# ntampellini/FIRECODE

Hardware: AMD Instinct MI355X
Metric: conformer-pair RMSD alignments/s (higher is better)
Workload: dtype f64

## Files before the change

### firecode_amd/_lib.py

```python

from __future__ import annotations

import ctypes as C
import os

import numpy as np

_HERE = os.path.dirname(os.path.abspath(__file__))
LIB_PATH = os.environ.get("FC_LIB_PATH") or os.path.join(_HERE, "libfc_hip.so")

FC_OK = 0
FC_E_INVALID, FC_E_NODEVICE, FC_E_HIP, FC_E_NOMEM, FC_E_LIMIT, FC_E_INTERNAL = -1, -2, -3, -4, -5, -6


class FirecodeHipError(RuntimeError):

    def __init__(self, code, message):
        super().__init__(f"libfc_hip error {code}: {message}")
        self.code = code


class FirecodeHipInputError(FirecodeHipError, ValueError):
    """FC_E_INVALID / FC_E_LIMIT: the arguments were rejected before any launch."""

# ... 76 lines not shown
    "fc_prune_export_pairs_dev": [_ens, C.c_void_p, _i64],
    "fc_prune_from_gathered_dev": [_ens, C.c_void_p, _i64, _i64, _i64, _p_u8, _p_i64],
    "fc_prune_from_gathered_dev_enqueue": [_ens, C.c_void_p, _i64, _i64, _i64, _i64, _i64],
    "fc_prune_collect": [_ens, _i64, _i64, _p_u8, _p_i64],
    "fc_stream_set": [C.c_void_p],
    "fc_memory_trim": [],
    "fc_host_alloc_pinned": [C.c_int64, C.POINTER(C.c_void_p)],
    "fc_host_free_pinned": [C.c_void_p],
    "fc_inertia_moments": [_p_f64, _i64, _i64, _p_f64, _p_f64],
    "fc_prune_rmsd_rot_corr": [_p_f64, _i64, _i64, _p_u8, _p_i64, _i64, _p_u8, _p_f64, C.POINTER(C.c_int32), _i64,
                               _f64, _f64, _p_f64, _f64, _i64, _p_u8, _p_u64],
    "fc_align_by_moi": [_p_f64, _i64, _i64, _p_f64, _p_f64],
    "fc_prune_moi": [_p_f64, _i64, _i64, _p_f64, _f64, _p_f64, _f64, _i64, _p_u8],
    "fc_moi_simbits": [_p_f64, _i64, _i64, _p_f64, _f64, _p_f64, _f64, _p_u64],
    "fc_align_to_first": [_p_f64, _i64, _i64, _p_i64, _i64, _p_f64],
    "fc_rototranslate": [_p_f64, _i64, _i64, _p_f64, _p_f64, _p_f64],
    "fc_clash_self": [_p_f64, _i64, _i64, _f64, _f64, _p_i64],
    "fc_clash_fragments": [_p_f64, _i64, _i64, _p_i64, _i64, _f64, _i64, _p_i64, _p_u8],
    "fc_clash_graph": [_p_f64, _i64, _i64, _p_u8, _f64, _p_i64],
    "fc_fitness_check": [_p_f64, _i64, _i64, _p_i64, _p_f64, _i64, _f64, _p_f64, _p_u8],
    "fc_bond_changes": [_p_f64, _i64, _i64, C.POINTER(C.c_int32), _i64, _p_f64, _p_f64, _i64, _p_u64, _p_i64, _p_i64,
                        _i64, _i64, _p_i64, _p_u8],
    "fc_bond_changes_list": [_p_f64, _i64, _i64, C.POINTER(C.c_int32), _i64, _p_f64, _p_f64, _i64, _p_u64, _p_i64,
                             _p_i64, _i64, _p_i64, _p_i64],
    "fc_embed_poses_clash": [_p_f64, _i64, _i64, _p_f64, _i64, _i64, _p_i64, _p_i64, _p_f64, _p_f64,
                             _p_f64, _p_f64, _i64, _f64, _i64, _p_i64, _p_u8, _p_f64],
    "fc_embed_mol_transforms": [_p_f64, _i64, _i64, _p_i64, _i64, _p_f64, _p_f64, _i64, _p_f64, _i64, _p_f64, _p_f64],
    "fc_embed_trimolecular": [C.POINTER(_p_f64), _p_i64, _p_i64, C.POINTER(_p_i64), _p_i64, _i64, _p_i64, _p_f64,
                              _p_f64, _p_f64, _p_f64, _p_u8, _p_i64, _p_f64, _p_f64, _i64, C.POINTER(C.c_int32),
                              _i64, _f64, _i64, _f64, _p_f64, _p_f64, _p_u8, _p_u8],
    "fc_embed_grid_clash": [_p_f64, _i64, _i64, _p_i64, _i64, _p_f64, _p_f64, _p_f64, _i64, _i64, _p_i64, _i64,
                            _p_f64, _p_f64, _p_f64, _i64, _p_f64, _i64, _f64, _i64, _p_u8,
                            C.POINTER(C.c_int32), _p_f64],
    "fc_embed_grid_dedupe": [_p_f64, _i64, _i64, _p_i64, _i64, _p_f64, _p_f64, _p_f64, _i64, _i64, _p_i64, _i64,
                             _p_f64, _p_f64, _p_f64, _i64, _p_f64, _i64, _f64, _i64, _f64, _p_u8, _p_u8],
    "fc_string_embed": [_p_f64, _i64, _i64, _p_f64, _p_f64, _i64, _p_f64, _i64, _i64, _p_f64, _p_f64, _i64, _p_f64, _i64,
                        _p_i64, _i64, _f64, _i64, _f64, _p_u8, _p_u8, _p_f64, _p_f64],
    "fc_torsion_scan": [_p_f64, _i64, _p_i64, _i64, _p_u8, _p_i64, _i64, _f64, _i64, _p_f64, _p_i64],
    "fc_torsion_scan_fingerprints": [_p_f64, _i64, _p_i64, _i64, _p_u8, _p_i64, _i64, _f64, _i64, _p_i64, _i64,
                                     _p_f64, _p_i64, _p_f64],
    "fc_torsion_scan_tfd": [_p_f64, _i64, _p_i64, _i64, _p_u8, _p_i64, _i64, _f64, _i64, _p_i64, _i64, _f64, _p_i64, _p_u8],
    "fc_torsion_scan_tfd_grid": [_p_f64, _i64, _p_i64, _i64, _p_u8, _p_i64, _p_i64, _f64, _i64, _p_i64, _i64, _f64, _p_i64, _p_u8],
    "fc_torsion_fingerprint": [_p_f64, _i64, _i64, _p_i64, _i64, _p_f64],
    "fc_tfd_simbits": [_p_f64, _i64, _i64, _f64, _i64, _i64, _p_u64],
    "fc_tfd_first_match": [_p_f64, _i64, _i64, _f64, _p_i64],
    "fc_tfd_last_form": [_p_i64],
    "fc_tfd_ladder_from_first_match": [_p_i64, _i64, _p_u8],
    "fc_tfd_prune": [_p_f64, _i64, _i64, _f64, _p_u8],
    "fc_debug_pyset_order_ints": [_p_i64, _i64, _p_i64, _p_i64],
    "fc_debug_pyset_order_pairs": [_p_i64, _i64, _p_i64, _p_i64],
    "fc_debug_pyset_order_pairs_device": [_p_i64, _i64, _p_i64],
    "fc_debug_tfd_ladder_emulate": [_p_i64, _i64, _p_u8],
    "fc_debug_ladder_from_pairs": [_p_u64, _i64, _i64, _i64, C.c_int, _i64, _p_u8, _p_i64],
    "fc_xyz_write": [C.c_char_p, C.POINTER(C.c_char_p), _i64, _p_f64, _i64, C.c_char_p, C.c_int],
    "fc_xyz_scan": [C.c_char_p, _p_i64, _p_i64],
    "fc_cartesian_product_i64": [_p_i64, _p_i64, _i64, _p_i64],
    "fc_cartesian_product_f64": [_p_f64, _p_i64, _i64, _p_f64],
    "fc_xyz_read": [C.c_char_p, _i64, _i64, C.c_char_p, _p_f64],
    "fc_bench_prune_rmsd": [_ens, _f64, _f64, _i64, _p_f64, _p_f64, _p_u8, _p_i64],
    "fc_stream_use": [C.c_void_p],
    "fc_ensemble_twin": [_ens, C.POINTER(_ens)],
    "fc_prune_rmsd_begin_split_async": [_ens, _f64, _f64, _i64, _i64, _i64, C.c_void_p, C.c_int],
    "fc_screen_last_kind": [],
    "fc_debug_screen_plan": [_i64, _i64, _i64, _i64, _f64, _f64, _i64, _p_i64],
    "fc_debug_mfma_f16_model": [_i64, _p_i64, _p_f64],
    "fc_debug_h2_covariance": [_ens, _i64, _i64, C.POINTER(C.c_float), _p_f64, _p_f64],
# ... 725 lines not shown
```

### firecode_amd/csrc/fc_api_geom.cpp

```cpp
#include "fc_internal.h"

using namespace fc;

extern "C" {

int fc_alignment_matrices(const double *p, const double *q, int64_t n_pairs, int64_t A,
                          double *M_out) {
  FC_API_LOCK;
  FC_REQUIRE(n_pairs >= 0 && A >= 1, "bad shape");
  if (n_pairs == 0) return FC_OK;
  FC_REQUIRE(p && q && M_out, "NULL pointer argument");
  FC_TRY(ensure_init());
  DevBuf dp, dq, dM;
  FC_TRY(upload(dp, p, (size_t)n_pairs * A * 3));
  FC_TRY(upload(dq, q, (size_t)n_pairs * A * 3));
  FC_TRY(dM.reserve((size_t)n_pairs * 9 * sizeof(double)));
  FC_TRY(launch_alignment_matrices(dp.as<double>(), dq.as<double>(), n_pairs, A, dM.as<double>()));
  FC_TRY(d2h(M_out, dM.p, (size_t)n_pairs * 9 * sizeof(double)));
  return sync();
}

int fc_align_by_moi(const double *coords, int64_t N, int64_t A, const double *masses, double *out) {
  FC_API_LOCK;
  FC_REQUIRE(N >= 0 && A >= 1, "bad shape");
// ... 362 lines not shown
    if (na1 * na2 * 4 * (int64_t)sizeof(int) > 64 * 1024)
      return set_error(FC_E_LIMIT, "na1*na2=%lld angle pairs per group exceed the 4096 of the LDS list",
                       (long long)(na1 * na2));
    FC_TRY(X2a.reserve(G2 * A2 * 3 * sizeof(double)));
    FC_TRY(dacc.reserve((size_t)P));
    FC_TRY(launch_embed_pretransform(d2.as<double>(), n2, A2, na2, R2.as<double>(), t2.as<double>(), 1, 0,
                                     X2a.as<double>()));
    FC_TRY(launch_embed_group_dedupe(X1.as<double>(), n1, A1, na1, X2a.as<double>(), n2, A2, na2, rmsd_thr,
                                     dpass.as<uint8_t>(), dacc.as<uint8_t>()));
    FC_TRY(d2h(accept_out, dacc.p, (size_t)P));
  }
  FC_TRY(d2h(pass_out, dpass.p, (size_t)P));
  if (counts_out) FC_TRY(d2h(counts_out, dcnt.p, (size_t)P * sizeof(int32_t)));
  FC_TRY(sync());
  if (ms_kernel) {
    float ms = 0.f;
    FC_HIP_TRY(hipEventElapsedTime(&ms, c.ev0, c.ev1));
    *ms_kernel = ms;
  }
  return FC_OK;
}

int fc_embed_grid_clash(const double *m1, int64_t n1, int64_t A1, const int64_t *reactive1,
                        int64_t nr1, const double *ps1, const double *pe1, const double *m2,
                        int64_t n2, int64_t A2, const int64_t *reactive2, int64_t nr2,
                        const double *ps2, const double *pe2, const double *angles1, int64_t na1,
                        const double *angles2, int64_t na2, double thresh, int64_t max_clashes,
                        uint8_t *pass_out, int32_t *counts_out, double *ms_kernel) {
  FC_API_LOCK;
  return embed_grid(m1, n1, A1, reactive1, nr1, ps1, pe1, m2, n2, A2, reactive2, nr2, ps2, pe2, angles1,
                    na1, angles2, na2, thresh, max_clashes, pass_out, counts_out, ms_kernel, 0.0, nullptr);
}

int fc_embed_grid_dedupe(const double *m1, int64_t n1, int64_t A1, const int64_t *reactive1,
                         int64_t nr1, const double *ps1, const double *pe1, const double *m2,
                         int64_t n2, int64_t A2, const int64_t *reactive2, int64_t nr2,
                         const double *ps2, const double *pe2, const double *angles1, int64_t na1,
                         const double *angles2, int64_t na2, double thresh, int64_t max_clashes,
                         double rmsd_thr, uint8_t *pass_out, uint8_t *accept_out) {
  FC_API_LOCK;
  FC_REQUIRE(accept_out != nullptr, "accept_out is NULL");
  return embed_grid(m1, n1, A1, reactive1, nr1, ps1, pe1, m2, n2, A2, reactive2, nr2, ps2, pe2, angles1,
                    na1, angles2, na2, thresh, max_clashes, pass_out, nullptr, nullptr, rmsd_thr, accept_out);
}

int fc_embed_trimolecular(const double *const coords[3], const int64_t n_conf[3], const int64_t n_atoms[3],
                          const int64_t *const reactive[3], const int64_t n_reactive[3], int64_t J,
                          const int64_t *conf, const double *piv_start, const double *piv_end,
                          const double *vecs, const double *dirs0, const uint8_t *run, const int64_t *rtab,
                          const double *norms, const double *ua, int64_t U, const int32_t *aidx, int64_t S,
                          double thresh, int64_t max_clashes, double rmsd_thr, double *dirs_out,
                          double *Rt_out, uint8_t *pass_out, uint8_t *accept_out) {
  FC_API_LOCK;
  FC_REQUIRE(coords && n_conf && n_atoms && reactive && n_reactive, "NULL pointer argument");
  FC_REQUIRE(J >= 0 && U >= 1 && S >= 1, "bad shape");
  if (J == 0) return FC_OK;
  FC_REQUIRE(conf && piv_start && piv_end && vecs && dirs0 && run && rtab && norms && ua && aidx && dirs_out &&
                 Rt_out && pass_out && accept_out,
             "NULL pointer argument");
  FC_REQUIRE(thresh > 0.0 && rmsd_thr > 0.0 && max_clashes >= 0, "thresholds must be positive");
  int64_t Atot = 0;
  for (int i = 0; i < 3; ++i) {
    FC_REQUIRE(coords[i] && reactive[i] && n_conf[i] >= 1 && n_atoms[i] >= 1, "bad molecule %d", i);
    FC_REQUIRE(n_reactive[i] >= 1 && n_reactive[i] <= 2, "molecule %d: 1 or 2 reactive atoms expected", i);
    for (int64_t r = 0; r < n_reactive[i]; ++r)
      FC_REQUIRE(reactive[i][r] >= 0 && reactive[i][r] < n_atoms[i], "reactive index out of range");
// ... 115 lines not shown
```

### firecode_amd/csrc/fc_embed.hip

```cpp
#include "fc_internal.h"
#include "fc_kabsch_math.h"

#include <algorithm>

namespace fc {

__device__ __forceinline__ void rot_axis_angle(double ax, double ay, double az, double angle_deg,
                                               double (&M)[9]) {
  double a2 = angle_deg / 2.0;
  a2 *= 3.141592653589793 / 180.0;
  double sn, cs;
  sincos(a2, &sn, &cs);
  const double nrm = sqrt((ax * ax + ay * ay) + az * az);
  const double q1 = sn * (ax / nrm), q2 = sn * (ay / nrm), q3 = sn * (az / nrm), q0 = cs;
  M[0] = 2.0 * (q0 * q0 + q1 * q1) - 1.0;
  M[1] = 2.0 * (q1 * q2 - q0 * q3);
  M[2] = 2.0 * (q1 * q3 + q0 * q2);
  M[3] = 2.0 * (q1 * q2 + q0 * q3);
  M[4] = 2.0 * (q0 * q0 + q2 * q2) - 1.0;
  M[5] = 2.0 * (q2 * q3 - q0 * q1);
  M[6] = 2.0 * (q1 * q3 - q0 * q2);
  M[7] = 2.0 * (q2 * q3 + q0 * q1);
  M[8] = 2.0 * (q0 * q0 + q3 * q3) - 1.0;
}
// ... 234 lines not shown
          const fc_f2 X = SX[ap], Y = SY[ap], Z = SZ[ap], Nn = SN[ap];
#pragma unroll
          for (int q = 0; q < NB; ++q) {
            fc_f2 v = __builtin_elementwise_fma(bz[q], Z, Nn);
            v = __builtin_elementwise_fma(by[q], Y, v);
            v = __builtin_elementwise_fma(bx[q], X, v);
            m[q] = fminf(fminf(m[q], v.x), v.y);
          }
        }
        if (scanning) {
#pragma unroll
          for (int q = NB - 1; q >= 0; --q)
            if (b0 + q < A2 && b0 + q >= resume && !(m[q] >= tb[q])) pending = b0 + q;
          if (pending < 0) resume = max(resume, min(b0 + NB, A2));
        }
      }
      if (pending >= 0) {
        const double ex = base2[(int64_t)(pending * 3 + 0) * S2 + s2];
        const double ey = base2[(int64_t)(pending * 3 + 1) * S2 + s2];
        const double ez = base2[(int64_t)(pending * 3 + 2) * S2 + s2];
        for (int a = 0; a < A1; ++a) {
          const double dx = ex - s[a * 3], dy = ey - s[a * 3 + 1], dz = ez - s[a * 3 + 2];
          const double d2 = ((dx * dx) + dy * dy) + dz * dz;
          cnt += (d2 < thr2) ? 1 : 0;
        }
        resume = (cnt > max_clashes) ? A2 : pending + 1;
      }
    }
    if (on) {
      const int64_t c2 = s2 / na2, a2 = s2 % na2;
      const int64_t p = ((c2 * n1 + c1) * 2 + o) * (na1 * na2) + (a2 * na1 + a1);
      pass[p] = (cnt <= max_clashes) ? 1 : 0;
      if (counts) counts[p] = cnt;
    }
  }
}

__global__ void __launch_bounds__(256)
k_string_transforms(const double *__restrict__ cen1, const double *__restrict__ vec1, int64_t n1,
                    int64_t K1, const double *__restrict__ cen2, const double *__restrict__ vec2,
                    int64_t n2, int64_t K2, const double *__restrict__ angles, int64_t nA,
                    double *__restrict__ R_out, double *__restrict__ t_out, int64_t *__restrict__ c1_out,
                    int64_t *__restrict__ c2_out) {
  const int64_t p = (int64_t)blockIdx.x * blockDim.x + threadIdx.x;
  const int64_t P = n1 * n2 * K1 * K2 * nA;
  if (p >= P) return;
  const int64_t ia = p % nA;
  const int64_t ki = (p / nA) % (K1 * K2);
  const int64_t ci = p / (nA * K1 * K2);
  const int64_t c1 = ci % n1, c2 = ci / n1, k1 = ki % K1, k2 = ki / K1;
  const double *p1 = cen1 + (c1 * K1 + k1) * 3, *rv = vec1 + (c1 * K1 + k1) * 3;
  const double *p2 = cen2 + (c2 * K2 + k2) * 3, *mv = vec2 + (c2 * K2 + k2) * 3;
  const double na = sqrt((mv[0] * mv[0] + mv[1] * mv[1]) + mv[2] * mv[2]);
  const double nb = sqrt((rv[0] * rv[0] + rv[1] * rv[1]) + rv[2] * rv[2]);
  const double ax = mv[0] / na, ay = mv[1] / na, az = mv[2] / na;
  const double bx = -rv[0] / nb, by = -rv[1] / nb, bz = -rv[2] / nb;
  const double vx = ay * bz - az * by, vy = az * bx - ax * bz, vz = ax * by - ay * bx;
  const double nv = sqrt((vx * vx + vy * vy) + vz * vz);
  double R[9] = {1, 0, 0, 0, 1, 0, 0, 0, 1};
  if (nv != 0.0) {
    const double c = (ax * bx + ay * by) + az * bz;
    const double f = (1.0 - c) / (nv * nv);
    const double k2m[9] = {(0.0 * 0.0 + -vz * vz) + vy * -vy, (0.0 * -vz + -vz * 0.0) + vy * vx, (0.0 * vy + -vz * -vx) + vy * 0.0,
                           (vz * 0.0 + 0.0 * vz) + -vx * -vy, (vz * -vz + 0.0 * 0.0) + -vx * vx, (vz * vy + 0.0 * -vx) + -vx * 0.0,
                           (-vy * 0.0 + vx * vz) + 0.0 * -vy, (-vy * -vz + vx * 0.0) + 0.0 * vx, (-vy * vy + vx * -vx) + 0.0 * 0.0};
    const double km[9] = {0.0, -vz, vy, vz, 0.0, -vx, -vy, vx, 0.0};
// ... 182 lines not shown
  const int64_t groups = n1 * n2 * 2;
  if (groups == 0) return FC_OK;
  int64_t blocks = ceil_div(groups, 4);
  const int64_t cap = (int64_t)ctx().n_cu * 8;
  if (blocks > cap) blocks = cap;
  hipLaunchKernelGGL(k_embed_group_dedupe, dim3((unsigned)blocks), dim3(256),
                     (size_t)4 * na1 * na2 * sizeof(int), ctx().stream, X1a, n1, (int)A1, na1, X2a, n2,
                     (int)A2, na2, thr, pass_dev, accept_dev);
  return check_launch("k_embed_group_dedupe");
}

int launch_embed_mol_transforms(const double *coords_dev, int64_t n, int64_t A,
                                const int64_t *reactive_dev, int nr, const double *ps_dev,
                                const double *pe_dev, int mol, const double *angles_dev, int64_t na,
                                double *R_dev, double *t_dev) {
  const int64_t total = n * 2 * na;
  if (total == 0) return FC_OK;
  hipLaunchKernelGGL(k_embed_mol_transforms, dim3((unsigned)ceil_div(total, 64)), dim3(64), 0,
                     ctx().stream, coords_dev, n, A, reactive_dev, nr, ps_dev, pe_dev, mol,
                     angles_dev, na, R_dev, t_dev);
  return check_launch("k_embed_mol_transforms");
}

int launch_embed_pretransform(const double *coords_dev, int64_t n, int64_t A, int64_t na,
                              const double *R_dev, const double *t_dev, int aos, int64_t S,
                              double *out_dev) {
  const int64_t total = n * 2 * na * A;
  if (total == 0) return FC_OK;
  hipLaunchKernelGGL(k_embed_pretransform, dim3((unsigned)ceil_div(total, 256)), dim3(256), 0,
                     ctx().stream, coords_dev, n, A, na, R_dev, t_dev, aos, S, out_dev);
  return check_launch("k_embed_pretransform");
}

int launch_embed_grid_clash(const double *X1_dev, int64_t n1, int64_t A1, int64_t na1,
                            const double *X2s_dev, int64_t n2, int64_t A2, int64_t na2, int64_t S2,
                            double thresh, int64_t max_clashes, void *scratch, size_t scratch_bytes,
                            uint8_t *pass_dev, int32_t *counts_dev) {
  const int64_t g1 = n1 * 2 * na1;
  if (g1 == 0 || n2 * na2 == 0) return FC_OK;
  const double thr2 = sq_threshold_lt(thresh);
  int64_t strips = ceil_div(S2, 256);
  const int64_t want = ceil_div((int64_t)ctx().n_cu * 16, g1);
  if (strips > want) strips = std::max<int64_t>(want, 1);
  const char *f64_env = getenv("FC_GRID_F64");
  if (f64_env && atoi(f64_env) == 1) {
    hipLaunchKernelGGL(k_embed_grid_clash_f64, dim3((unsigned)g1, (unsigned)strips), dim3(256),
                       (size_t)A1 * 3 * sizeof(double), ctx().stream, X1_dev, n1, (int)A1, na1, X2s_dev,
                       n2, (int)A2, na2, S2, thr2, (int)max_clashes, (int)strips, pass_dev, counts_dev);
    return check_launch("k_embed_grid_clash_f64");
  }
  const int64_t len1 = g1 * A1 * 3, len2 = 2 * A2 * 3 * S2;
  if (scratch_bytes < 256 + (size_t)len2 * sizeof(float)) return set_error(FC_E_INVALID, "pose grid scratch too small");
  auto *scratch_dev = static_cast<unsigned long long *>(scratch);
  float *X2f_dev = reinterpret_cast<float *>(static_cast<char *>(scratch) + 256);
  FC_HIP_TRY(hipMemsetAsync(scratch_dev, 0, sizeof(unsigned long long), ctx().stream));
  hipLaunchKernelGGL(k_to_f32, dim3((unsigned)ceil_div(len2, 256)), dim3(256), 0, ctx().stream, X2s_dev, len2, X2f_dev);
  hipLaunchKernelGGL(k_max_abs, dim3((unsigned)std::min<int64_t>(ceil_div(len1, 256), 1024)), dim3(256), 0,
                     ctx().stream, X1_dev, len1, scratch_dev);
  hipLaunchKernelGGL(k_max_abs, dim3((unsigned)std::min<int64_t>(ceil_div(len2, 256), 1024)), dim3(256), 0,
                     ctx().stream, X2s_dev, len2, scratch_dev);
  FC_TRY(check_launch("k_max_abs"));
  const size_t lds = (size_t)A1 * 3 * sizeof(double) + (size_t)4 * ((A1 + 1) / 2) * sizeof(fc_f2);
  hipLaunchKernelGGL(k_embed_grid_clash, dim3((unsigned)g1, (unsigned)strips), dim3(256), lds, ctx().stream,
                     X1_dev, n1, (int)A1, na1, X2s_dev, n2, (int)A2, na2, S2, thr2, (int)max_clashes,
                     (int)strips, scratch_dev, X2f_dev, pass_dev, counts_dev);
  return check_launch("k_embed_grid_clash");
}

__global__ void k_warm_embed() {}
int warm_embed() {
  hipLaunchKernelGGL(k_warm_embed, dim3(1), dim3(64), 0, ctx().stream);
  return check_launch("k_warm_embed");
}

}
```

### firecode_amd/csrc/fc_internal.h

```cpp
#pragma once

#include "fc_common.h"

namespace fc {

int prebuild_screen_items(fc_ensemble *e);
int launch_rmsd_values(fc_ensemble *e, double small_rmsd, double *rmsd_dev, double *maxdev_dev, int64_t rank = 0,
                       int64_t world = 1, bool explicit_sum = false);
int launch_gather_matrix_pairs(const double *rmsd_m, const double *maxdev_m, int64_t N, const int64_t *pi_dev,
                               const int64_t *pj_dev, int64_t P, double *rmsd_out, double *maxdev_out);
int launch_mirror_upper(double *m_dev, int64_t N);
int launch_scatter_pairs(const uint64_t *pairs_dev, int64_t n_pairs, int64_t N, int64_t W, uint64_t *bits_dev);
int launch_prep_begin(fc_ensemble *e);
int launch_prep_body(const double *coords_dev, int64_t N, int64_t A_all, const int32_t *sel_dev, int64_t A, int center,
                     fc_ensemble *e, const int32_t *conf_idx_dev);
int launch_pairs_exact(const fc_ensemble *e, const int64_t *pi_dev, const int64_t *pj_dev, int64_t P, double *rmsd_dev,
                       double *maxdev_dev, double *R_dev, bool inverted = false);
int launch_matrix_exact(const fc_ensemble *e, double *rmsd_dev, double *maxdev_dev);
int last_screen_kind();
void screen_select(int kind);
int ensure_h2_operands(fc_ensemble *e, double *scale_out);
int launch_simbits_screen(fc_ensemble *e, double thr2_margin);
int debug_screen_plan(int64_t N, int64_t A, int64_t row_block, bool lean, double g_max, double max_rmsd, int h2_model,
                      int64_t plan_out[5]);
// ... 68 lines not shown
int warm_clash();
int launch_torsion_scan(const double *base_dev, int64_t A, const int64_t *torsions_dev, int64_t T,
                        const uint8_t *rotmasks_dev, const int16_t *mv_dev, const int16_t *rs_dev,
                        const int32_t *nmv_dev, const int32_t *nrs_dev, const int64_t *angles_dev, int64_t S,
                        double thresh, int64_t backoff, double *out_dev, int64_t *rot_dev, const int64_t *quads_dev,
                        int64_t Q, double *tf_dev);
int launch_rotcorr_simbits(const double *X_dev, int64_t N, int64_t A, const uint8_t *heavy_dev, const int64_t *tors_dev,
                           int64_t T, const uint8_t *rotmasks_dev, const double *angles_dev,
                           const int32_t *n_angles_dev, int max_angles, double max_rmsd, double max_dev,
                           const double *energies_dev, double max_dE, uint64_t *bits_dev, int64_t W);
int launch_torsion_fingerprint(const double *coords_dev, int64_t N, int64_t A, const int64_t *quads_dev, int64_t Q,
                               double *tf_dev);
int launch_angle_grid(const int64_t *values_dev, const int64_t *first_dev, const int64_t *counts_dev, int64_t T,
                      int64_t S, int64_t *out_dev);
int launch_rows_to_sets(const int64_t *idx_dev, const int64_t *rows_dev, int64_t n, int64_t *out_dev);
int launch_select_rotated(const int64_t *rot_dev, int64_t S, int64_t *idx_dev, int64_t *count_dev, DevBuf &tmp);
int warm_torsion();
int launch_string_transforms(const double *cen1, const double *vec1, int64_t n1, int64_t K1, const double *cen2,
                             const double *vec2, int64_t n2, int64_t K2, const double *angles, int64_t nA,
                             double *R_dev, double *t_dev, int64_t *c1_dev, int64_t *c2_dev);
int launch_pose_fingerprints(const double *m1, int64_t A1, const double *m2, int64_t A2, const int64_t *c1,
                             const int64_t *c2, const double *R2, const double *t2, int64_t P, const int64_t *quads,
                             int64_t Q, const uint8_t *pass, double *tf);
int launch_embed_group_dedupe(const double *X1a, int64_t n1, int64_t A1, int64_t na1, const double *X2a, int64_t n2,
                              int64_t A2, int64_t na2, double thr, const uint8_t *pass_dev, uint8_t *accept_dev);
int launch_embed_mol_transforms(const double *coords_dev, int64_t n, int64_t A, const int64_t *reactive_dev, int nr,
                                const double *ps_dev, const double *pe_dev, int mol, const double *angles_dev,
                                int64_t na, double *R_dev, double *t_dev);
int launch_embed_pretransform(const double *coords_dev, int64_t n, int64_t A, int64_t na, const double *R_dev,
                              const double *t_dev, int aos, int64_t S, double *out_dev);
int launch_embed_grid_clash(const double *X1_dev, int64_t n1, int64_t A1, int64_t na1, const double *X2s_dev,
                            int64_t n2, int64_t A2, int64_t na2, int64_t S2, double thresh, int64_t max_clashes,
                            void *scratch, size_t scratch_bytes, uint8_t *pass_dev, int32_t *counts_dev);
int warm_embed();
size_t tri_group_lds_bytes(int64_t Atot, int U, int S);
int launch_tri_embed(const double *const coords_dev[3], const int64_t *const reactive_dev[3], const int64_t A[3],
                     const int64_t nr[3], int64_t J, const int64_t *conf_dev, const double *piv_start_dev,
                     const double *piv_end_dev, const double *vecs_dev, const double *dirs0_dev, const uint8_t *run_dev,
                     const int64_t *rtab_dev, const double *norms_dev, const double *ua_dev, int U,
                     const int32_t *aidx_dev, int S, double thresh, int max_clashes, double rmsd_thr, double *dirs_dev,
                     double *Rt_dev, uint8_t *pass_dev, uint8_t *accept_dev);
int warm_embed3();
struct SymTable {
  const uint16_t *perms_dev = nullptr;
  int K = 1;
  bool mirror = false;
  unsigned long long *stats_dev = nullptr;
};
int diverse_lanes(int64_t N);
size_t diverse_sym_lds_bytes(int64_t A, int64_t K);
int select_diverse(fc_ensemble *e, int64_t n_max, int64_t start, double stop_rmsd, int64_t *indices_out,
                   double *radii_out, int32_t *labels_out, double *dist_out, int64_t *n_selected, double *ms_device,
                   const SymTable *sym = nullptr);
int warm_diverse();
struct ClusterGraph {
  const uint64_t *pairs_dev = nullptr;
  const unsigned long long *n_pairs_dev = nullptr;
  unsigned long long n_pairs_host = 0;
  bool known_short = false;
  const unsigned long long *n_cand_dev = nullptr;
  unsigned long long cand_cap = 0;
  const unsigned long long *redo_dev = nullptr;
  const uint64_t *bits_dev = nullptr;
  int64_t W = 0;
};
constexpr int kClStatusErr = 0;
// ... 136 lines not shown
```

### firecode_amd/csrc/fc_tuning.h

```cpp
#pragma once

#if !defined(FC_TUNING_BUILD) &&                                                                                             \
    (defined(FC_TIMELINE) || defined(FC_H2_TIMELINE) || defined(FC_RB_TIMELINE) || defined(FC_TFD_STAMPS) || defined(FC_TFD_STAMPS_SMALL) || defined(FC_H2_ABLATE_K) ||   \
     defined(FC_H2_ABLATE_ROWS) || defined(FC_H2_ABLATE_POLY) || defined(FC_F32_ABLATE_K) || defined(FC_F32_ABLATE_POLY) ||  \
     defined(FC_ABLATE_PUSH) || defined(FC_ABLATE_STAGE) || defined(FC_ABLATE_OVERFLOW) || defined(FC_ABLATE_REDO) ||         \
     defined(FC_RB_NOSTAGE) || defined(FC_RB_NOPASS1) || defined(FC_RB_NOPASS2) || defined(FC_RB_NOJACOBI) ||                \
     defined(FC_RB_NOCOMPUTE) || defined(FC_RB_ROWS_FROM_LDS) || defined(FC_RB_SAMEROW) || defined(FC_RB_WPS) ||              \
     defined(FC_RB_AHEAD) || defined(FC_RB_CHUNK) || defined(FC_H2_WGS) || defined(FC_F32_WGS) || defined(FC_REFINE_ROUNDS) || defined(FC_STAGE_PAIRS_F32) || defined(FC_TS_WGS) || defined(FC_TS_TURN) || defined(FC_KNN_SYM_ROWS))
#error "a tuning switch (FC_*TIMELINE / FC_*ABLATE* / FC_RB_* / FC_TFD_STAMPS ...) without -DFC_TUNING_BUILD: see fc_tuning.h"
#endif

#ifdef __cplusplus
namespace fc {
constexpr int64_t kDiverseLanes8MaxN = 10000;
constexpr int kKnnWorkgroupsPerCu = 4;
constexpr int kKnnMaxStrips = 64;
constexpr int kButinaRounds = 16;
constexpr long long kButinaLiveEdges = 1ll << 22;
}
#endif
```

### firecode_amd/embeds.py

```python

import numpy as np

from firecode_amd import _lib as L


def rototranslate(coords, R, t):
    X, R, t = L.f64(coords), L.f64(R), L.f64(t)
    if X.ndim != 3 or R.shape != (X.shape[0], 3, 3) or t.shape != (X.shape[0], 3):
        raise L.FirecodeHipInputError(L.FC_E_INVALID, "coords (n, A, 3), R (n, 3, 3), t (n, 3) expected")
    out = np.empty_like(X)
    L.call("fc_rototranslate", L.pf(X), X.shape[0], X.shape[1], L.pf(R), L.pf(t), L.pf(out))
    return out


def get_embed(mols, conf_ids):
    return np.concatenate([
        rototranslate(L.f64(mol.coords[c])[None], L.f64(mol.rotation)[None], L.f64(mol.position)[None])[0]
        for mol, c in zip(mols, conf_ids)
    ])


def embed_poses_clash(m1, m2, c1, c2, R1, t1, R2, t2, thresh=1.5, max_clashes=0, return_poses=False):
    m1, m2 = L.f64(m1), L.f64(m2)
    c1, c2 = L.i64(c1), L.i64(c2)
# ... 22 lines not shown
    return X, r, np.ascontiguousarray(pv[:, 0]), np.ascontiguousarray(pv[:, 1])


def embed_mol_transforms(coords, reactive, pivots, mol, angles):
    X, r, ps, pe = _mol_args(coords, reactive, pivots)
    ang = L.f64(angles).reshape(-1)
    n, na = X.shape[0], ang.shape[0]
    R = np.empty((n, 2, na, 3, 3))
    t = np.empty((n, 2, na, 3))
    L.call("fc_embed_mol_transforms", L.pf(X), n, X.shape[1], L.pi(r), r.shape[0], L.pf(ps), L.pf(pe),
           int(mol), L.pf(ang), na, L.pf(R), L.pf(t))
    return R, t


def embed_grid_clash(m1, reactive1, pivots1, m2, reactive2, pivots2, angles1, angles2=None,
                     thresh=1.5, max_clashes=0, return_counts=False):
    import ctypes as C

    X1, r1, ps1, pe1 = _mol_args(m1, reactive1, pivots1)
    X2, r2, ps2, pe2 = _mol_args(m2, reactive2, pivots2)
    a1 = L.f64(angles1).reshape(-1)
    a2 = a1 if angles2 is None else L.f64(angles2).reshape(-1)
    shape = (X2.shape[0], X1.shape[0], 2, a2.shape[0], a1.shape[0])
    ok = np.zeros(shape, dtype=np.uint8)
    counts = np.zeros(shape, dtype=np.int32) if return_counts else None
    ms = C.c_double(0)
    L.call("fc_embed_grid_clash", L.pf(X1), X1.shape[0], X1.shape[1], L.pi(r1), r1.shape[0], L.pf(ps1), L.pf(pe1),
           L.pf(X2), X2.shape[0], X2.shape[1], L.pi(r2), r2.shape[0], L.pf(ps2), L.pf(pe2),
           L.pf(a1), a1.shape[0], L.pf(a2), a2.shape[0], float(thresh), int(max_clashes), L.pb(ok),
           None if counts is None else counts.ctypes.data_as(C.POINTER(C.c_int32)), C.byref(ms))
    if return_counts:
        return ok.view(np.bool_), counts, ms.value
    return ok.view(np.bool_), ms.value


def embed_grid_poses(m1, reactive1, pivots1, m2, reactive2, pivots2, angles1, angles2=None,
                     thresh=1.5, max_clashes=0, rmsd_thr=1.0):
    X1, r1, ps1, pe1 = _mol_args(m1, reactive1, pivots1)
    X2, r2, ps2, pe2 = _mol_args(m2, reactive2, pivots2)
    a1 = L.f64(angles1).reshape(-1)
    a2 = a1 if angles2 is None else L.f64(angles2).reshape(-1)
    shape = (X2.shape[0], X1.shape[0], 2, a2.shape[0], a1.shape[0])
    ok = np.zeros(shape, dtype=np.uint8)
    acc = np.zeros(shape, dtype=np.uint8)
    L.call("fc_embed_grid_dedupe", L.pf(X1), X1.shape[0], X1.shape[1], L.pi(r1), r1.shape[0], L.pf(ps1), L.pf(pe1),
           L.pf(X2), X2.shape[0], X2.shape[1], L.pi(r2), r2.shape[0], L.pf(ps2), L.pf(pe2),
           L.pf(a1), a1.shape[0], L.pf(a2), a2.shape[0], float(thresh), int(max_clashes), float(rmsd_thr),
           L.pb(ok), L.pb(acc))
    return acc.view(np.bool_), ok.view(np.bool_)


def string_embed_poses(m1, centers1, orbvecs1, m2, centers2, orbvecs2, angles, quadruplets,
                       thresh=1.5, max_clashes=0, tfd_thresh=10):
    X1, X2 = L.f64(m1), L.f64(m2)
    c1, v1, c2, v2 = (L.f64(a) for a in (centers1, orbvecs1, centers2, orbvecs2))
    ang = L.f64(angles).reshape(-1)
    quads = L.i64(quadruplets).reshape(-1, 4)
    n1, n2, K1, K2, nA = X1.shape[0], X2.shape[0], c1.shape[1], c2.shape[1], ang.shape[0]
    if c1.shape != (n1, K1, 3) or v1.shape != c1.shape or c2.shape != (n2, K2, 3) or v2.shape != c2.shape:
        raise L.FirecodeHipInputError(L.FC_E_INVALID, "centers/orbvecs must be (n_conf, K, 3)")
    P = n1 * n2 * K1 * K2 * nA
    ok = np.zeros(P, dtype=np.uint8)
    acc = np.zeros(P, dtype=np.uint8)
    R2 = np.empty((P, 3, 3))
    t2 = np.empty((P, 3))
    L.call("fc_string_embed", L.pf(X1), n1, X1.shape[1], L.pf(c1), L.pf(v1), K1, L.pf(X2), n2, X2.shape[1],
# ... 267 lines not shown
```

### include/fc_hip.h

```cpp
#ifndef FC_HIP_H
#define FC_HIP_H

#include <stdint.h>

#ifdef __cplusplus
extern "C" {
#endif

#define FC_OK 0
#define FC_E_INVALID (-1)
#define FC_E_NODEVICE (-2)
#define FC_E_HIP (-3)
#define FC_E_NOMEM (-4)
#define FC_E_LIMIT (-5)
#define FC_E_INTERNAL (-6)

int fc_abi_version(void);
int fc_device_count(void);
int fc_init(int device);
int fc_shutdown(void);
const char *fc_last_error(void);
int fc_warmup(void);
int fc_stream_set(void *hip_stream);
int fc_stream_use(void *hip_stream);
// ... 169 lines not shown
                       int64_t n_ids, double thresh, int64_t max_clashes,
                       int64_t *counts_out, uint8_t *pass_out);

int fc_clash_graph(const double *coords, int64_t N, int64_t A, const uint8_t *adj, double thresh,
                   int64_t *counts_out);
int fc_bond_changes(const double *coords, int64_t N, int64_t A, const int32_t *atom_class, int64_t n_class,
                    const double *class_thresh, const double *ref_coords, int64_t ref_stride, const uint64_t *ref_bits,
                    const int64_t *excl_offsets, const int64_t *excl_atoms, int64_t excl_sets, int64_t max_newbonds,
                    int64_t *counts_out, uint8_t *ok_out);
int fc_bond_changes_list(const double *coords, int64_t N, int64_t A, const int32_t *atom_class, int64_t n_class,
                         const double *class_thresh, const double *ref_coords, int64_t ref_stride,
                         const uint64_t *ref_bits, const int64_t *excl_offsets, const int64_t *excl_atoms,
                         int64_t excl_sets, const int64_t *offsets, int64_t *bonds_out);
int fc_fitness_check(const double *coords, int64_t N, int64_t A, const int64_t *pairs,
                     const double *targets, int64_t C, double threshold, double *error_out,
                     uint8_t *pass_out);

int fc_embed_poses_clash(const double *m1, int64_t n1, int64_t A1, const double *m2,
                         int64_t n2, int64_t A2, const int64_t *c1, const int64_t *c2,
                         const double *R1, const double *t1, const double *R2,
                         const double *t2, int64_t P, double thresh, int64_t max_clashes,
                         int64_t *counts_out, uint8_t *pass_out, double *poses_out);

int fc_embed_mol_transforms(const double *coords, int64_t n, int64_t A, const int64_t *reactive,
                            int64_t nr, const double *pivot_start, const double *pivot_end,
                            int64_t mol, const double *angles, int64_t na, double *R_out,
                            double *t_out);
int fc_embed_grid_clash(const double *m1, int64_t n1, int64_t A1, const int64_t *reactive1,
                        int64_t nr1, const double *ps1, const double *pe1, const double *m2,
                        int64_t n2, int64_t A2, const int64_t *reactive2, int64_t nr2,
                        const double *ps2, const double *pe2, const double *angles1, int64_t na1,
                        const double *angles2, int64_t na2, double thresh, int64_t max_clashes,
                        uint8_t *pass_out, int32_t *counts_out, double *ms_kernel);
int fc_embed_grid_dedupe(const double *m1, int64_t n1, int64_t A1, const int64_t *reactive1,
                         int64_t nr1, const double *ps1, const double *pe1, const double *m2,
                         int64_t n2, int64_t A2, const int64_t *reactive2, int64_t nr2,
                         const double *ps2, const double *pe2, const double *angles1, int64_t na1,
                         const double *angles2, int64_t na2, double thresh, int64_t max_clashes,
                         double rmsd_thr, uint8_t *pass_out, uint8_t *accept_out);

int fc_embed_trimolecular(const double *const coords[3], const int64_t n_conf[3], const int64_t n_atoms[3],
                          const int64_t *const reactive[3], const int64_t n_reactive[3], int64_t J,
                          const int64_t *conf, const double *piv_start, const double *piv_end,
                          const double *vecs, const double *dirs0, const uint8_t *run, const int64_t *rtab,
                          const double *norms, const double *ua, int64_t U, const int32_t *aidx, int64_t S,
                          double thresh, int64_t max_clashes, double rmsd_thr, double *dirs_out,
                          double *Rt_out, uint8_t *pass_out, uint8_t *accept_out);

int fc_string_embed(const double *m1, int64_t n1, int64_t A1, const double *centers1,
                    const double *orbvecs1, int64_t K1, const double *m2, int64_t n2, int64_t A2,
                    const double *centers2, const double *orbvecs2, int64_t K2,
                    const double *angles, int64_t nA, const int64_t *quads, int64_t Q,
                    double thresh, int64_t max_clashes, double tfd_thresh, uint8_t *pass_out,
                    uint8_t *accept_out, double *R2_out, double *t2_out);

int fc_torsion_scan(const double *base, int64_t A, const int64_t *torsions, int64_t T,
                    const uint8_t *rotmasks, const int64_t *angles, int64_t S, double thresh,
                    int64_t backoff_deg, double *coords_out, int64_t *rotated_bonds_out);
int fc_torsion_scan_fingerprints(const double *base, int64_t A, const int64_t *torsions, int64_t T,
                                 const uint8_t *rotmasks, const int64_t *angles, int64_t S, double thresh,
                                 int64_t backoff_deg, const int64_t *quads, int64_t Q, double *tf_out,
                                 int64_t *rotated_bonds_out, double *coords_out);
int fc_torsion_scan_tfd(const double *base, int64_t A, const int64_t *torsions, int64_t T, const uint8_t *rotmasks,
                        const int64_t *angles, int64_t S, double thresh, int64_t backoff_deg, const int64_t *quads,
                        int64_t Q, double tfd_thresh, int64_t *rotated_bonds_out, uint8_t *keep_out);
int fc_torsion_scan_tfd_grid(const double *base, int64_t A, const int64_t *torsions, int64_t T, const uint8_t *rotmasks,
// ... 69 lines not shown
```

Before: 19.95 billion.

## Add bounding-sphere culled grid clash kernel with compacted candidate lists

```diff
diff --git a/firecode_amd/_lib.py b/firecode_amd/_lib.py
--- a/firecode_amd/_lib.py
+++ b/firecode_amd/_lib.py
@@ -132,6 +132,7 @@
     "fc_embed_grid_clash": [_p_f64, _i64, _i64, _p_i64, _i64, _p_f64, _p_f64, _p_f64, _i64, _i64, _p_i64, _i64,
                             _p_f64, _p_f64, _p_f64, _i64, _p_f64, _i64, _f64, _i64, _p_u8,
                             C.POINTER(C.c_int32), _p_f64],
+    "fc_debug_grid_cull_stats": [_i64, _p_i64],
     "fc_embed_grid_dedupe": [_p_f64, _i64, _i64, _p_i64, _i64, _p_f64, _p_f64, _p_f64, _i64, _i64, _p_i64, _i64,
                              _p_f64, _p_f64, _p_f64, _i64, _p_f64, _i64, _f64, _i64, _f64, _p_u8, _p_u8],
     "fc_string_embed": [_p_f64, _i64, _i64, _p_f64, _p_f64, _i64, _p_f64, _i64, _i64, _p_f64, _p_f64, _i64, _p_f64, _i64,
diff --git a/firecode_amd/csrc/fc_api_geom.cpp b/firecode_amd/csrc/fc_api_geom.cpp
--- a/firecode_amd/csrc/fc_api_geom.cpp
+++ b/firecode_amd/csrc/fc_api_geom.cpp
@@ -418,6 +418,13 @@
                     na1, angles2, na2, thresh, max_clashes, pass_out, counts_out, ms_kernel, 0.0, nullptr);
 }
 
+int fc_debug_grid_cull_stats(int64_t arm, int64_t *out4) {
+  FC_API_LOCK;
+  if (arm != 0) grid_cull_stats_arm();
+  if (out4 != nullptr) grid_cull_stats_get(out4);
+  return FC_OK;
+}
+
 int fc_embed_grid_dedupe(const double *m1, int64_t n1, int64_t A1, const int64_t *reactive1,
                          int64_t nr1, const double *ps1, const double *pe1, const double *m2,
                          int64_t n2, int64_t A2, const int64_t *reactive2, int64_t nr2,
diff --git a/firecode_amd/csrc/fc_embed.hip b/firecode_amd/csrc/fc_embed.hip
--- a/firecode_amd/csrc/fc_embed.hip
+++ b/firecode_amd/csrc/fc_embed.hip
@@ -290,6 +290,234 @@
       const int64_t p = ((c2 * n1 + c1) * 2 + o) * (na1 * na2) + (a2 * na1 + a1);
       pass[p] = (cnt <= max_clashes) ? 1 : 0;
       if (counts) counts[p] = cnt;
+    }
+  }
+}
+
+#ifndef FC_GRID_CULL_NB
+#define FC_GRID_CULL_NB 8
+#endif
+#ifndef FC_GRID_CULL_PB
+#define FC_GRID_CULL_PB 8
+#endif
+#ifndef FC_GRID_CULL_FIT
+#define FC_GRID_CULL_FIT 1
+#endif
+__device__ __forceinline__ void wave_lds_order() {
+  __builtin_amdgcn_fence(__ATOMIC_RELEASE, "wavefront");
+  __builtin_amdgcn_wave_barrier();
+  __builtin_amdgcn_fence(__ATOMIC_ACQUIRE, "wavefront");
+}
+
+template <int NB>
+__device__ __forceinline__ void grid_cull_scan_round(const uint16_t *list, int n_items, int base, int lane,
+                                                     const float *__restrict__ base2f, int64_t S2, int64_t s2w, float Tf,
+                                                     const fc_f2 *SX, const fc_f2 *SY, const fc_f2 *SZ, const fc_f2 *SN,
+                                                     int P1, unsigned long long *sus_wave) {
+  fc_f2 bx[NB], by[NB], bz[NB];
+  float m[NB], tb[NB];
+  int item[NB];
+#pragma unroll
+  for (int q = 0; q < NB; ++q) {
+    const int idx = base + q * 64 + lane;
+    item[q] = idx < n_items ? (int)list[idx] : -1;
+    const int it = item[q] < 0 ? (int)list[n_items - 1] : item[q];
+    const int64_t at = s2w + (it & 63);
+    const int b = it >> 6;
+    const float x = base2f[(int64_t)(b * 3 + 0) * S2 + at];
+    const float y = base2f[(int64_t)(b * 3 + 1) * S2 + at];
+    const float z = base2f[(int64_t)(b * 3 + 2) * S2 + at];
+    bx[q] = fc_f2{x, x}, by[q] = fc_f2{y, y}, bz[q] = fc_f2{z, z};
+    tb[q] = Tf - fmaf(x, x, fmaf(y, y, z * z));
+    m[q] = 3.0e38f;
+  }
+  for (int ap = 0; ap < P1; ++ap) {
+    const fc_f2 X = SX[ap], Y = SY[ap], Z = SZ[ap], Nn = SN[ap];
+#pragma unroll
+    for (int q = 0; q < NB; ++q) {
+      fc_f2 v = __builtin_elementwise_fma(bz[q], Z, Nn);
+      v = __builtin_elementwise_fma(by[q], Y, v);
+      v = __builtin_elementwise_fma(bx[q], X, v);
+      m[q] = fminf(fminf(m[q], v.x), v.y);
+    }
+  }
+#pragma unroll
+  for (int q = 0; q < NB; ++q)
+    if (item[q] >= 0 && !(m[q] >= tb[q])) atomicOr(&sus_wave[item[q] & 63], 1ull << (item[q] >> 6));
+}
+
+__global__ void __launch_bounds__(256)
+k_embed_grid_clash_cull(const double *__restrict__ X1, int64_t n1, int A1, int64_t na1,
+                        const double *__restrict__ X2s, int64_t n2, int A2, int64_t na2, int64_t S2,
+                        double thr2, int max_clashes, int strips, const unsigned long long *__restrict__ maxabs,
+                        const float *__restrict__ X2f, uint8_t *__restrict__ pass, int32_t *__restrict__ counts,
+                        unsigned long long *__restrict__ stats) {
+  constexpr int NB = FC_GRID_CULL_NB;
+  constexpr int PB = FC_GRID_CULL_PB;
+  extern __shared__ double s[];
+  const int tid = threadIdx.x, lane = tid & 63, wave = tid >> 6;
+  const int P1 = (A1 + 1) / 2;
+  fc_f2 *SX = reinterpret_cast<fc_f2 *>(s + A1 * 3), *SY = SX + P1, *SZ = SY + P1, *SN = SZ + P1;
+  unsigned long long *sus = reinterpret_cast<unsigned long long *>(SN + P1);
+  uint16_t *list = reinterpret_cast<uint16_t *>(sus + 256) + (size_t)wave * 64 * A2;
+  const int64_t g1 = blockIdx.x;
+  const int64_t a1 = g1 % na1;
+  const int o = (int)((g1 / na1) % 2);
+  const int64_t c1 = g1 / (2 * na1);
+  for (int k = tid; k < A1 * 3; k += 256) s[k] = X1[g1 * (int64_t)A1 * 3 + k];
+  for (int k = tid; k < P1 * 2; k += 256) {
+    const bool real = k < A1;
+    const double *src = X1 + g1 * (int64_t)A1 * 3 + (int64_t)k * 3;
+    const float x = real ? (float)src[0] : 0.f, y = real ? (float)src[1] : 0.f, z = real ? (float)src[2] : 0.f;
+    reinterpret_cast<float *>(SX)[k] = -2.f * x;
+    reinterpret_cast<float *>(SY)[k] = -2.f * y;
+    reinterpret_cast<float *>(SZ)[k] = -2.f * z;
+    reinterpret_cast<float *>(SN)[k] = real ? (float)(((double)x * x + (double)y * y) + (double)z * z) : 3.0e37f;
+  }
+  __syncthreads();
+  double *red = reinterpret_cast<double *>(sus);
+  float cxf, cyf, czf;
+  bool finite = true;
+  {
+    double sx = 0.0, sy = 0.0, sz = 0.0;
+    for (int k = tid; k < A1; k += 256) {
+      const float x = (float)s[k * 3], y = (float)s[k * 3 + 1], z = (float)s[k * 3 + 2];
+      finite = finite && isfinite(x) && isfinite(y) && isfinite(z);
+      sx += (double)x, sy += (double)y, sz += (double)z;
+    }
+    for (int off = 32; off > 0; off >>= 1) {
+      sx += __shfl_xor(sx, off), sy += __shfl_xor(sy, off), sz += __shfl_xor(sz, off);
+    }
+    finite = __all(finite);
+    if (lane == 0) red[wave * 4] = sx, red[wave * 4 + 1] = sy, red[wave * 4 + 2] = sz, red[wave * 4 + 3] = finite ? 1.0 : 0.0;
+    __syncthreads();
+    cxf = (float)((((red[0] + red[4]) + red[8]) + red[12]) / (double)A1);
+    cyf = (float)((((red[1] + red[5]) + red[9]) + red[13]) / (double)A1);
+    czf = (float)((((red[2] + red[6]) + red[10]) + red[14]) / (double)A1);
+    finite = red[3] != 0.0 && red[7] != 0.0 && red[11] != 0.0 && red[15] != 0.0;
+  }
+  double r2 = 0.0;
+  for (int k = tid; k < A1; k += 256) {
+    const double dx = (double)(float)s[k * 3] - (double)cxf, dy = (double)(float)s[k * 3 + 1] - (double)cyf,
+                 dz = (double)(float)s[k * 3 + 2] - (double)czf;
+    const double d2 = ((dx * dx) + dy * dy) + dz * dz;
+    if (d2 > r2) r2 = d2;
+  }
+  for (int off = 32; off > 0; off >>= 1) {
+    const double other = __shfl_xor(r2, off);
+    if (other > r2) r2 = other;
+  }
+  if (lane == 0) red[16 + wave] = r2;
+  __syncthreads();
+  r2 = fmax(fmax(red[16], red[17]), fmax(red[18], red[19]));
+  __syncthreads();
+  float Tf, boundf;
+  bool cull;
+  {
+    const double M = __longlong_as_double((long long)maxabs[0]);
+    const double thr = sqrt(thr2) * (1.0 + 0x1p-40);
+    const double e0 = M * 0x1p-24;
+    double T = thr2 + 2.0 * ((2.0 * thr * 3.47 * e0 + 12.0 * e0 * e0) + (30.0 + 16.0) * M * M * 0x1p-24);
+    T *= 1.0 + 0x1p-20;
+    Tf = nextafterf((float)T, INFINITY);
+    if (!(M < 1.0e15)) Tf = INFINITY;
+    const double rho = sqrt(r2) * (1.0 + 0x1p-40);
+    const double reach = (rho + thr) + 2.0 * 3.47 * e0;
+    const double B = (reach * reach) * (1.0 + 0x1p-20);
+    boundf = nextafterf((float)B, INFINITY);
+    cull = finite && M < 1.0e15 && B > 1.0e-30 && B < 1.0e37;
+  }
+  const int64_t n_s2 = n2 * na2;
+  const double *__restrict__ base2 = X2s + (int64_t)o * A2 * 3 * S2;
+  const float *__restrict__ base2f = X2f + (int64_t)o * A2 * 3 * S2;
+  unsigned long long st_kept = 0, st_rec = 0;
+  for (int64_t s2 = (int64_t)blockIdx.y * 256 + tid; s2 < S2; s2 += (int64_t)strips * 256) {
+    const bool on = s2 < n_s2;
+    const int64_t s2w = s2 - lane;
+    sus[tid] = 0ull;
+    int n_items = 0;
+    const float *__restrict__ row =
+        X2f + (int64_t)__builtin_amdgcn_readfirstlane(o) * A2 * 3 * S2 +
+        (((int64_t)__builtin_amdgcn_readfirstlane((int)(s2w >> 32)) << 32) |
+         (int64_t)(uint32_t)__builtin_amdgcn_readfirstlane((int)(uint32_t)s2w));
+    for (int b0 = 0; b0 < A2; b0 += PB) {
+      float x[PB], y[PB], z[PB];
+#pragma unroll
+      for (int q = 0; q < PB; ++q) {
+        x[q] = row[lane];
+        y[q] = row[S2 + lane];
+        z[q] = row[2 * S2 + lane];
+        if (b0 + q + 1 < A2) row += 3 * S2;
+      }
+#pragma unroll
+      for (int q = 0; q < PB; ++q) {
+        const float dx = x[q] - cxf, dy = y[q] - cyf, dz = z[q] - czf;
+        const float d2 = fmaf(dx, dx, fmaf(dy, dy, dz * dz));
+        const bool keep = on && b0 + q < A2 && !(cull && d2 >= boundf);
+        const uint64_t mask = __ballot(keep);
+        const int before = (int)__builtin_amdgcn_mbcnt_hi((uint32_t)(mask >> 32), __builtin_amdgcn_mbcnt_lo((uint32_t)mask, 0u));
+        if (keep) list[n_items + before] = (uint16_t)(lane | ((b0 + q) << 6));
+        n_items += __popcll(mask);
+      }
+    }
+    wave_lds_order();
+#define FC_CULL_ROUND(nb) \
+  grid_cull_scan_round<nb>(list, n_items, base, lane, base2f, S2, s2w, Tf, SX, SY, SZ, SN, P1, sus + wave * 64)
+#ifdef FC_GRID_CULL_ABLATE_SCAN
+    n_items = 0;
+#endif
+    int base = 0;
+    for (; n_items - base > (FC_GRID_CULL_FIT ? (NB - 1) * 64 : 0); base += NB * 64) FC_CULL_ROUND(NB);
+    if (FC_GRID_CULL_FIT && base < n_items) {
+      switch ((n_items - base + 63) / 64) {
+        case 1: FC_CULL_ROUND(1); break;
+        case 2: FC_CULL_ROUND(2); break;
+        case 3: FC_CULL_ROUND(3); break;
+        case 4: FC_CULL_ROUND(4); break;
+        case 5: FC_CULL_ROUND(5); break;
+        case 6: FC_CULL_ROUND(6); break;
+        default: FC_CULL_ROUND(7); break;
+      }
+    }
+#undef FC_CULL_ROUND
+    wave_lds_order();
+    unsigned long long w = sus[tid];
+    int cnt = 0;
+#ifdef FC_GRID_CULL_ABLATE_RECOUNT
+    w = 0ull;
+#endif
+    while (w != 0ull && cnt <= max_clashes) {
+      const int b = __ffsll((long long)w) - 1;
+      w &= w - 1ull;
+      const double ex = base2[(int64_t)(b * 3 + 0) * S2 + s2];
+      const double ey = base2[(int64_t)(b * 3 + 1) * S2 + s2];
+      const double ez = base2[(int64_t)(b * 3 + 2) * S2 + s2];
+      for (int a = 0; a < A1; ++a) {
+        const double dx = ex - s[a * 3], dy = ey - s[a * 3 + 1], dz = ez - s[a * 3 + 2];
+        const double d2 = ((dx * dx) + dy * dy) + dz * dz;
+        cnt += (d2 < thr2) ? 1 : 0;
+      }
+      ++st_rec;
+    }
+    if (on) {
+      int64_t c2, a2;
+      if (S2 <= 0x7fffffff) {
+        c2 = (int64_t)((uint32_t)s2 / (uint32_t)na2), a2 = (int64_t)((uint32_t)s2 % (uint32_t)na2);
+      } else {
+        c2 = s2 / na2, a2 = s2 % na2;
+      }
+      const int64_t p = ((c2 * n1 + c1) * 2 + o) * (na1 * na2) + (a2 * na1 + a1);
+      pass[p] = (cnt <= max_clashes) ? 1 : 0;
+      if (counts) counts[p] = cnt;
+    }
+    if (lane == 0) st_kept += (unsigned long long)n_items;
+    wave_lds_order();
+  }
+  if (stats) {
+    for (int off = 32; off > 0; off >>= 1) st_rec += __shfl_xor(st_rec, off);
+    if (lane == 0) {
+      atomicAdd(&stats[0], st_kept);
+      atomicAdd(&stats[1], st_rec);
     }
   }
 }
@@ -538,6 +766,29 @@
   return check_launch("k_embed_pretransform");
 }
 
+static size_t grid_cull_lds(int64_t A1, int64_t A2) {
+  return (size_t)A1 * 3 * sizeof(double) + (size_t)4 * ((A1 + 1) / 2) * sizeof(fc_f2) + 256 * sizeof(unsigned long long) +
+         (size_t)4 * 64 * A2 * sizeof(uint16_t);
+}
+
+bool grid_cull_fits(int64_t A1, int64_t A2) { return A2 <= 64 && grid_cull_lds(A1, A2) <= (size_t)64 * 1024; }
+
+static bool g_cull_armed = false;
+static int64_t g_cull_stats[4] = {-1, 0, 0, 0};
+
+void grid_cull_stats_arm() { g_cull_armed = true; }
+void grid_cull_stats_get(int64_t *out4) {
+  for (int k = 0; k < 4; ++k) out4[k] = g_cull_stats[k];
+}
+
+static void grid_cull_stats_plain(int kernel, int64_t n_s2, int64_t g1, int64_t A2) {
+  if (!g_cull_armed) return;
+  g_cull_armed = false;
+  g_cull_stats[0] = kernel;
+  g_cull_stats[1] = g_cull_stats[2] = n_s2 * g1 * A2;
+  g_cull_stats[3] = -1;
+}
+
 int launch_embed_grid_clash(const double *X1_dev, int64_t n1, int64_t A1, int64_t na1,
                             const double *X2s_dev, int64_t n2, int64_t A2, int64_t na2, int64_t S2,
                             double thresh, int64_t max_clashes, void *scratch, size_t scratch_bytes,
@@ -553,23 +804,44 @@
     hipLaunchKernelGGL(k_embed_grid_clash_f64, dim3((unsigned)g1, (unsigned)strips), dim3(256),
                        (size_t)A1 * 3 * sizeof(double), ctx().stream, X1_dev, n1, (int)A1, na1, X2s_dev,
                        n2, (int)A2, na2, S2, thr2, (int)max_clashes, (int)strips, pass_dev, counts_dev);
+    grid_cull_stats_plain(2, n2 * na2, g1, A2);
     return check_launch("k_embed_grid_clash_f64");
   }
   const int64_t len1 = g1 * A1 * 3, len2 = 2 * A2 * 3 * S2;
   if (scratch_bytes < 256 + (size_t)len2 * sizeof(float)) return set_error(FC_E_INVALID, "pose grid scratch too small");
   auto *scratch_dev = static_cast<unsigned long long *>(scratch);
   float *X2f_dev = reinterpret_cast<float *>(static_cast<char *>(scratch) + 256);
-  FC_HIP_TRY(hipMemsetAsync(scratch_dev, 0, sizeof(unsigned long long), ctx().stream));
+  FC_HIP_TRY(hipMemsetAsync(scratch_dev, 0, 128, ctx().stream));
   hipLaunchKernelGGL(k_to_f32, dim3((unsigned)ceil_div(len2, 256)), dim3(256), 0, ctx().stream, X2s_dev, len2, X2f_dev);
   hipLaunchKernelGGL(k_max_abs, dim3((unsigned)std::min<int64_t>(ceil_div(len1, 256), 1024)), dim3(256), 0,
                      ctx().stream, X1_dev, len1, scratch_dev);
   hipLaunchKernelGGL(k_max_abs, dim3((unsigned)std::min<int64_t>(ceil_div(len2, 256), 1024)), dim3(256), 0,
                      ctx().stream, X2s_dev, len2, scratch_dev);
   FC_TRY(check_launch("k_max_abs"));
+  const char *cull_env = getenv("FC_GRID_CULL");
+  if (!(cull_env && atoi(cull_env) == 0) && grid_cull_fits(A1, A2)) {
+    unsigned long long *stats_dev = g_cull_armed ? scratch_dev + 8 : nullptr;
+    hipLaunchKernelGGL(k_embed_grid_clash_cull, dim3((unsigned)g1, (unsigned)strips), dim3(256), grid_cull_lds(A1, A2),
+                       ctx().stream, X1_dev, n1, (int)A1, na1, X2s_dev, n2, (int)A2, na2, S2, thr2, (int)max_clashes,
+                       (int)strips, scratch_dev, X2f_dev, pass_dev, counts_dev, stats_dev);
+    FC_TRY(check_launch("k_embed_grid_clash_cull"));
+    if (stats_dev) {
+      g_cull_armed = false;
+      unsigned long long got[2] = {0, 0};
+      FC_HIP_TRY(hipMemcpyAsync(got, stats_dev, sizeof(got), hipMemcpyDeviceToHost, ctx().stream));
+      FC_HIP_TRY(hipStreamSynchronize(ctx().stream));
+      g_cull_stats[0] = 1;
+      g_cull_stats[1] = (int64_t)got[0];
+      g_cull_stats[2] = n2 * na2 * g1 * A2;
+      g_cull_stats[3] = (int64_t)got[1];
+    }
+    return FC_OK;
+  }
   const size_t lds = (size_t)A1 * 3 * sizeof(double) + (size_t)4 * ((A1 + 1) / 2) * sizeof(fc_f2);
   hipLaunchKernelGGL(k_embed_grid_clash, dim3((unsigned)g1, (unsigned)strips), dim3(256), lds, ctx().stream,
                      X1_dev, n1, (int)A1, na1, X2s_dev, n2, (int)A2, na2, S2, thr2, (int)max_clashes,
                      (int)strips, scratch_dev, X2f_dev, pass_dev, counts_dev);
+  grid_cull_stats_plain(0, n2 * na2, g1, A2);
   return check_launch("k_embed_grid_clash");
 }
 
diff --git a/firecode_amd/csrc/fc_internal.h b/firecode_amd/csrc/fc_internal.h
--- a/firecode_amd/csrc/fc_internal.h
+++ b/firecode_amd/csrc/fc_internal.h
@@ -124,6 +124,9 @@
 int launch_embed_grid_clash(const double *X1_dev, int64_t n1, int64_t A1, int64_t na1, const double *X2s_dev,
                             int64_t n2, int64_t A2, int64_t na2, int64_t S2, double thresh, int64_t max_clashes,
                             void *scratch, size_t scratch_bytes, uint8_t *pass_dev, int32_t *counts_dev);
+bool grid_cull_fits(int64_t A1, int64_t A2);
+void grid_cull_stats_arm();
+void grid_cull_stats_get(int64_t *out4);
 int warm_embed();
 size_t tri_group_lds_bytes(int64_t Atot, int U, int S);
 int launch_tri_embed(const double *const coords_dev[3], const int64_t *const reactive_dev[3], const int64_t A[3],
diff --git a/firecode_amd/csrc/fc_tuning.h b/firecode_amd/csrc/fc_tuning.h
--- a/firecode_amd/csrc/fc_tuning.h
+++ b/firecode_amd/csrc/fc_tuning.h
@@ -6,7 +6,9 @@
      defined(FC_ABLATE_PUSH) || defined(FC_ABLATE_STAGE) || defined(FC_ABLATE_OVERFLOW) || defined(FC_ABLATE_REDO) ||         \
      defined(FC_RB_NOSTAGE) || defined(FC_RB_NOPASS1) || defined(FC_RB_NOPASS2) || defined(FC_RB_NOJACOBI) ||                \
      defined(FC_RB_NOCOMPUTE) || defined(FC_RB_ROWS_FROM_LDS) || defined(FC_RB_SAMEROW) || defined(FC_RB_WPS) ||              \
-     defined(FC_RB_AHEAD) || defined(FC_RB_CHUNK) || defined(FC_H2_WGS) || defined(FC_F32_WGS) || defined(FC_REFINE_ROUNDS) || defined(FC_STAGE_PAIRS_F32) || defined(FC_TS_WGS) || defined(FC_TS_TURN) || defined(FC_KNN_SYM_ROWS))
+     defined(FC_RB_AHEAD) || defined(FC_RB_CHUNK) || defined(FC_H2_WGS) || defined(FC_F32_WGS) || defined(FC_REFINE_ROUNDS) || defined(FC_STAGE_PAIRS_F32) || defined(FC_TS_WGS) || defined(FC_TS_TURN) || defined(FC_KNN_SYM_ROWS) ||   \
+     defined(FC_GRID_CULL_NB) || defined(FC_GRID_CULL_FIT) || defined(FC_GRID_CULL_PB) ||        \
+     defined(FC_GRID_CULL_ABLATE_SCAN) || defined(FC_GRID_CULL_ABLATE_RECOUNT))
 #error "a tuning switch (FC_*TIMELINE / FC_*ABLATE* / FC_RB_* / FC_TFD_STAMPS ...) without -DFC_TUNING_BUILD: see fc_tuning.h"
 #endif
 
diff --git a/firecode_amd/embeds.py b/firecode_amd/embeds.py
--- a/firecode_amd/embeds.py
+++ b/firecode_amd/embeds.py
@@ -78,6 +78,15 @@
     if return_counts:
         return ok.view(np.bool_), counts, ms.value
     return ok.view(np.bool_), ms.value
+
+
+GRID_KERNELS = {-1: None, 0: "screen", 1: "cull", 2: "f64"}
+
+
+def grid_cull_stats(arm=False):
+    out = np.zeros(4, dtype=np.int64)
+    L.call("fc_debug_grid_cull_stats", int(bool(arm)), L.pi(out))
+    return {"kernel": GRID_KERNELS[int(out[0])], "kept": int(out[1]), "possible": int(out[2]), "recounted": int(out[3])}
 
 
 def embed_grid_poses(m1, reactive1, pivots1, m2, reactive2, pivots2, angles1, angles2=None,
diff --git a/include/fc_hip.h b/include/fc_hip.h
--- a/include/fc_hip.h
+++ b/include/fc_hip.h
@@ -225,6 +225,7 @@
                         const double *ps2, const double *pe2, const double *angles1, int64_t na1,
                         const double *angles2, int64_t na2, double thresh, int64_t max_clashes,
                         uint8_t *pass_out, int32_t *counts_out, double *ms_kernel);
+int fc_debug_grid_cull_stats(int64_t arm, int64_t *out4);
 int fc_embed_grid_dedupe(const double *m1, int64_t n1, int64_t A1, const int64_t *reactive1,
                          int64_t nr1, const double *ps1, const double *pe1, const double *m2,
                          int64_t n2, int64_t A2, const int64_t *reactive2, int64_t nr2,
```

New measurement: 20.00 billion (median of 2 runs). No clear change (+0.2%).
